# josefmaierfl/matchinglib_poselib

Hardware: AMD Instinct MI355X
Metric: descriptor-pairs/s (8k x 8k ORB BF-Hamming kNN=2 + ratio) (higher is better)
Workload: dtype fp4 (E2M1 MFMA, f32 accumulate: exact); 1 GPU; C2: 8192x8192 ORB-256 BF-Hamming kNN=2 + 0.75 ratio + DMatch rows, 64 image pair(s) per GPU per step; pairs_per_gpu=64, settle_steps=400, solver_polish=1

## Files before the change

### include/mlpl_debug.h

```cpp
#ifndef MLPL_DEBUG_H
#define MLPL_DEBUG_H
#include "mlpl_c.h"

#ifdef __cplusplus
extern "C" {
#endif

int mlpl_debug_arrsac_trace(mlpl_ctx *ctx, int32_t *buf, int cap);

int mlpl_debug_usac_trace(mlpl_ctx *ctx, double *buf, int cap_records);

int mlpl_debug_ransac_draw(mlpl_ctx *ctx, long long out[2]);

long long mlpl_debug_fiber_selftest(int n, int workers, int rounds);

int mlpl_debug_eig9(mlpl_ctx *ctx, const double *G, const double *start, int count, double *out12, double *jacobi10);

int mlpl_debug_dk_stats(mlpl_ctx *ctx, int enable, int stats[16]);

int mlpl_debug_l2_flags(mlpl_ctx *ctx, int flags[4]);

int mlpl_debug_hamming_stamps(mlpl_ctx *ctx, unsigned long long *out, int max_items);

int mlpl_debug_hamming_clock(mlpl_ctx *ctx, unsigned long long *out, int max_items);

int mlpl_debug_hop_trace(mlpl_ctx *ctx, float *us, int *codes, int max_items, long long *ws_grows);

int mlpl_debug_last_kernels(mlpl_ctx *ctx, int out[13]);

int mlpl_debug_last_hamming_top2(mlpl_ctx *ctx);

int mlpl_debug_last_l2_match(mlpl_ctx *ctx, int out[4]);

int mlpl_debug_l2_fold_counts(mlpl_ctx *ctx, const float *d_q, int nq, size_t q_stride, size_t q_batch_stride, const float *d_t, int nt,
                              size_t t_stride, size_t t_batch_stride, int dim, int ratio_test, float ratio, int batch, int32_t *d_idx, float *d_dist,
                              int32_t *counts);

int mlpl_debug_count_pass(mlpl_ctx *ctx, const double *p1, const double *p2, int n, const double *E, int n_live, int n_bound,
                          const int32_t *ids, int table_len, double thresh2, int point_splits, int32_t *table_inout);

#ifdef __cplusplus
}
#endif
#endif
```

### matchinglib_poselib_amd/_lib.py

```python
from __future__ import annotations

import ctypes as C
import os
import threading

_HERE = os.path.dirname(os.path.abspath(__file__))
_LIB_PATH = os.environ.get("MLPL_LIB_PATH") or os.path.join(_HERE, "lib", "libmlpl_hip.so")

MLPL_OK = 0
MLPL_E_BAD_INPUT = -1
MLPL_E_UNSUPPORTED = -2
MLPL_E_FAILED = -3
MLPL_E_INTERNAL = -103
MLPL_E_FEW_KEYPOINTS = -4
MLPL_E_NO_DEVICE = -100
MLPL_E_HIP = -101
MLPL_E_NOMEM = -102


class MlplError(RuntimeError):
    def __init__(self, code: int, where: str, msg: str = ""):
        self.code = code
        super().__init__(f"{where} failed with code {code}: {msg}")

# ... 77 lines not shown
    "mlpl_usac_essential_dev": (c_int, [c_void_p, c_void_p, c_void_p, c_int, c_void_p, c_void_p, c_void_p, c_void_p, c_void_p]),
    "mlpl_usac_essential_batch_dev": (c_int, [c_void_p, c_int, c_void_p, c_void_p, c_int, c_void_p, c_void_p, c_void_p, c_void_p, c_void_p, c_void_p,
                                              c_void_p, c_void_p, c_int, c_void_p, c_void_p]),
    "mlpl_usac_last_stats": (c_int, [c_void_p, c_void_p]),
    "mlpl_usac_last_degeneracy": (c_int, [c_void_p, c_void_p, c_void_p, c_void_p, c_int]),
    "mlpl_debug_usac_trace": (c_int, [c_void_p, c_void_p, c_int]),
    "mlpl_ransac_essential": (c_int, [c_void_p, c_void_p, c_void_p, c_int, c_double, c_double, c_int, c_int, c_u32,
                                      c_void_p, c_void_p, C.POINTER(c_int), C.POINTER(c_int)]),
    "mlpl_ransac_essential_dev": (c_int, [c_void_p, c_void_p, c_void_p, c_int, c_double, c_double, c_int, c_int,
                                          c_u32, c_void_p, c_void_p, C.POINTER(c_int), C.POINTER(c_int), c_void_p]),
    "mlpl_solve_5pt": (c_int, [c_void_p, c_void_p, c_void_p, c_int, c_void_p, c_int, c_void_p, c_void_p]),
    "mlpl_score_models": (c_int, [c_void_p, c_void_p, c_void_p, c_int, c_void_p, c_int, c_double, c_void_p,
                                  c_void_p]),
    "mlpl_ransac_last_stats": (c_int, [c_void_p, c_void_p]),
    "mlpl_debug_ransac_draw": (c_int, [c_void_p, c_void_p]),
    "mlpl_debug_fiber_selftest": (C.c_longlong, [c_int, c_int, c_int]),
    "mlpl_debug_eig9": (c_int, [c_void_p, c_void_p, c_void_p, c_int, c_void_p, c_void_p]),
    "mlpl_debug_dk_stats": (c_int, [c_void_p, c_int, c_void_p]),
    "mlpl_debug_hamming_stamps": (c_int, [c_void_p, c_void_p, c_int]),
    "mlpl_debug_hamming_clock": (c_int, [c_void_p, c_void_p, c_int]),
    "mlpl_debug_hop_trace": (c_int, [c_void_p, c_void_p, c_void_p, c_int, c_void_p]),
    "mlpl_debug_last_kernels": (c_int, [c_void_p, c_void_p]),
    "mlpl_debug_last_hamming_top2": (c_int, [c_void_p]),
    "mlpl_debug_count_pass": (c_int, [c_void_p, c_void_p, c_void_p, c_int, c_void_p, c_int, c_int, c_void_p, c_int, c_double, c_int,
                                      c_void_p]),
    "mlpl_pair_pose_dev": (c_int, [c_void_p, c_void_p, c_int, c_void_p, c_int, c_int, c_void_p, c_void_p, c_void_p, c_void_p, c_double,
                                   c_int, c_double, c_int, c_u32, c_double, c_void_p, c_void_p]),
    "mlpl_pair_pose_batch_dev": (c_int, [c_void_p, c_int, c_void_p, c_int, c_void_p, c_int, c_int, c_void_p, c_void_p, c_void_p, c_void_p, c_double,
                                         c_int, c_double, c_int, c_void_p, c_double, c_void_p, c_void_p, c_void_p]),
    "mlpl_pair_pose_f32_dev": (c_int, [c_void_p, c_void_p, c_int, c_void_p, c_int, c_int, c_void_p, c_void_p, c_void_p, c_void_p, c_double,
                                       c_int, c_double, c_int, c_u32, c_double, c_void_p, c_void_p]),
    "mlpl_pair_pose_batch_f32_dev": (c_int, [c_void_p, c_int, c_void_p, c_int, c_void_p, c_int, c_int, c_void_p, c_void_p, c_void_p, c_void_p, c_double,
                                             c_int, c_double, c_int, c_void_p, c_double, c_void_p, c_void_p, c_void_p]),
    "mlpl_pair_pose_batch_usac_f32_dev": (c_int, [c_void_p, c_int, c_void_p, c_int, c_void_p, c_int, c_int, c_void_p, c_void_p, c_void_p, c_void_p, c_void_p, c_int,
                                                  c_void_p, c_double, c_void_p, c_void_p, c_void_p]),
    "mlpl_pair_pose_batch_arrsac_f32_dev": (c_int, [c_void_p, c_int, c_void_p, c_int, c_void_p, c_int, c_int, c_void_p, c_void_p, c_void_p, c_void_p, c_double, c_int,
                                                    c_void_p, c_double, c_void_p, c_void_p, c_void_p]),
    "mlpl_pair_pose_batch_lanes_dev": (c_int, [c_void_p, c_void_p, c_int, c_int, c_void_p, c_int, c_void_p, c_int, c_int, c_void_p, c_void_p, c_void_p, c_void_p,
                                               c_double, c_int, c_double, c_void_p, c_double, c_void_p, c_void_p, c_void_p]),
    "mlpl_pair_pose_batch_usac_dev": (c_int, [c_void_p, c_int, c_void_p, c_int, c_void_p, c_int, c_int, c_void_p, c_void_p, c_void_p, c_void_p, c_void_p, c_int,
                                              c_void_p, c_double, c_void_p, c_void_p, c_void_p]),
    "mlpl_pair_pose_batch_arrsac_dev": (c_int, [c_void_p, c_int, c_void_p, c_int, c_void_p, c_int, c_int, c_void_p, c_void_p, c_void_p, c_void_p, c_double, c_int,
                                                c_void_p, c_double, c_void_p, c_void_p, c_void_p]),
    "mlpl_sorted_match_idx": (c_int, [c_void_p, c_int, c_void_p]),
    "mlpl_pair_batch_last_stats": (c_int, [c_void_p, c_void_p]),
    "mlpl_ransac_essential_batch_dev": (c_int, [c_void_p, c_int, c_void_p, c_void_p, c_int, c_void_p, c_double, c_int, c_double, c_void_p, c_int, c_double,
# ... 118 lines not shown
        check(self._lib.mlpl_ctx_synchronize(self._h), "mlpl_ctx_synchronize")

    def set_option(self, name: str, value: int):
        check(self._lib.mlpl_set_option(self._h, name.encode(), int(value)), "mlpl_set_option")

    def get_option(self, name: str) -> int:
        v = C.c_int(0)
        check(self._lib.mlpl_get_option(self._h, name.encode(), C.byref(v)), "mlpl_get_option")
        return v.value

    def last_kernels(self) -> list:
        out = (C.c_int * 13)()
        n = self._lib.mlpl_debug_last_kernels(self._h, out)
        if n < 0:
            raise MlplError(n, "mlpl_debug_last_kernels", last_error())
        return list(out[:n])

    def last_hamming_top2(self) -> int:
        n = self._lib.mlpl_debug_last_hamming_top2(self._h)
        if n < 0:
            raise MlplError(n, "mlpl_debug_last_hamming_top2", last_error())
        return n

    def last_l2_match(self) -> list:
        out = (C.c_int * 4)()
        n = self._lib.mlpl_debug_last_l2_match(self._h, out)
        if n < 0:
            raise MlplError(n, "mlpl_debug_last_l2_match", last_error())
        return list(out[:n])

    def close(self):
        if getattr(self, "_h", None) is not None and self._h:
            self._lib.mlpl_ctx_destroy(self._h)
            self._h = None

    def __del__(self):
        try:
            self.close()
        except Exception:
            pass

    def __enter__(self):
        return self

    def __exit__(self, *exc):
        self.close()
# ... 15 lines not shown
```

### matchinglib_poselib_amd/csrc/capi.hip

```cpp

#include <algorithm>
#include <cfloat>
#include <cstdlib>
#include <cstring>
#include <new>

#include "mlpl_internal.h"

namespace mlpl {

static thread_local char g_err[512] = "";

void set_error(const char *fmt, ...) {
    va_list ap;
    va_start(ap, fmt);
    vsnprintf(g_err, sizeof(g_err), fmt, ap);
    va_end(ap);
}

int ws_get(mlpl_ctx *ctx, WsSlot slot, size_t bytes, void **out) {
    if (bytes < 4096) bytes = 4096;
    if (ctx->ws_bytes[slot] < bytes) {
        MLPL_HIP_TRY(hipDeviceSynchronize());
        if (ctx->ws[slot]) MLPL_HIP_TRY(hipFree(ctx->ws[slot]));
// ... 91 lines not shown
    hipDeviceProp_t prop;
    MLPL_HIP_TRY(hipGetDeviceProperties(&prop, device_ordinal));
    if (std::strncmp(prop.gcnArchName, "gfx950", 6) != 0) {
        set_error("device %d is %s; this library carries gfx950 code objects only", device_ordinal, prop.gcnArchName);
        return MLPL_E_NO_DEVICE;
    }
    mlpl_ctx *ctx = new (std::nothrow) mlpl_ctx();
    if (!ctx) return MLPL_E_NOMEM;
    std::memset(ctx, 0, sizeof(*ctx));
    ctx->device = device_ordinal;
    ctx->num_cus = prop.multiProcessorCount > 0 ? prop.multiProcessorCount : 256;
    ctx->opt_hamming_variant = 3;
    ctx->opt_hamming_qpl = 1;
    ctx->opt_hamming_blocks_per_cu = 32;
    ctx->opt_hamming_mfma_blocks_per_cu = 3;
    ctx->opt_hamming_mfma_qt = 0;
    ctx->opt_hamming_mfma_lds = 1;
    ctx->opt_hamming_mfma_weighted = 1;
    ctx->opt_hamming_mfma_prio = 0;
    ctx->opt_hamming_fused_merge = 1;
    ctx->opt_hamming_expand_fine = 1;
    ctx->opt_hamming_expand_inkernel = 1;
    ctx->opt_hamming_block_top2 = 4;
    ctx->opt_hamming_merge_emit = 0;
    ctx->opt_ransac_lazy_sums = 1;
    ctx->opt_ransac_overlap = 1;
    ctx->opt_ransac_f32_filter = 1;
    ctx->opt_ransac_count_mpl = 2;
    ctx->opt_ransac_count_tiles = 2;
    ctx->opt_ransac_count_wpe = 5;
    ctx->opt_ransac_count_threads = 256;
    ctx->opt_ransac_count_defer = 1;
    ctx->opt_pair_batch_feed = 1;
    ctx->opt_solver_polish = 1;
    ctx->opt_solver_wave3 = 1;
    ctx->opt_ransac_device_draw = 1;
    ctx->opt_usac_lo_warm_start = 1;
    ctx->opt_usac_lo5_fused_fit = 1;
    ctx->opt_hub_blocking_sync = 1;
    ctx->opt_eig_inverse_iteration = 1;
    ctx->opt_arrsac_refine_warm_start = 1;
    ctx->opt_usac_sprt_fast = 1;
    ctx->opt_l2_float_mfma = 1;
    ctx->opt_l2_fold_counts = 1;
    ctx->opt_vfc_store_u = 0;
    hipError_t e = hipStreamCreateWithFlags(&ctx->stream, hipStreamNonBlocking);
// ... 41 lines not shown
    for (int i = 0; i < 2; ++i)
        if (ctx->aux_stream[i]) (void)hipStreamDestroy(ctx->aux_stream[i]);
    for (int i = 0; i < 8; ++i)
        if (ctx->aux_ev[i]) (void)hipEventDestroy(ctx->aux_ev[i]);
    delete ctx;
}

void *mlpl_ctx_stream(mlpl_ctx *ctx) { return ctx ? (void *)ctx->stream : nullptr; }
int mlpl_ctx_device(mlpl_ctx *ctx) { return ctx ? ctx->device : -1; }
int mlpl_ctx_synchronize(mlpl_ctx *ctx) {
    if (!ctx) return MLPL_E_BAD_INPUT;
    MLPL_HIP_TRY(hipStreamSynchronize(ctx->stream));
    return MLPL_OK;
}

static const struct {
    const char *name;
    int mlpl_ctx::*field;
    int lo, hi;
} kRangeOptions[] = {
    {"l2_fold_counts", &mlpl_ctx::opt_l2_fold_counts, 0, 1},
    {"hamming_expand_inkernel", &mlpl_ctx::opt_hamming_expand_inkernel, 0, 1},
    {"hamming_block_top2", &mlpl_ctx::opt_hamming_block_top2, 0, 4},
    {"vfc_store_u", &mlpl_ctx::opt_vfc_store_u, 0, 1},
};

int mlpl_set_option(mlpl_ctx *ctx, const char *name, int value) {
    if (!ctx || !name) return MLPL_E_BAD_INPUT;
    for (const auto &o : kRangeOptions)
        if (!std::strcmp(name, o.name)) {
            const bool bad_block = o.field == &mlpl_ctx::opt_hamming_block_top2 && value != 0 && value != 4;
            if (value < o.lo || value > o.hi || bad_block) {
                set_error("mlpl_set_option: unknown option or bad value: %s=%d", name, value);
                return MLPL_E_BAD_INPUT;
            }
            ctx->*(o.field) = value;
            return MLPL_OK;
        }
    if (!std::strcmp(name, "hamming_variant") && value >= 0 && value <= 3) ctx->opt_hamming_variant = value;
    else if (!std::strcmp(name, "hamming_mfma_qt") && (value == 0 || value == 1 || value == 2 || value == 4)) ctx->opt_hamming_mfma_qt = value;
    else if (!std::strcmp(name, "hamming_mfma_blocks_per_cu") && value >= 1 && value <= 64) ctx->opt_hamming_mfma_blocks_per_cu = value;
    else if (!std::strcmp(name, "hamming_mfma_lds") && (value >= 0 && value <= 2)) ctx->opt_hamming_mfma_lds = value;
    else if (!std::strcmp(name, "hamming_expand_fine") && (value == 0 || value == 1)) ctx->opt_hamming_expand_fine = value;
    else if (!std::strcmp(name, "hamming_mfma_prio") && (value == 0 || value == 1 || value == 3)) ctx->opt_hamming_mfma_prio = value;
    else if (!std::strcmp(name, "hamming_mfma_prefetch") && (value == 0 || value == 2 || value == 4 || value == 6)) ctx->opt_hamming_mfma_prefetch = value;
    else if (!std::strcmp(name, "hamming_split_rows") && (value == 0 || value == 4096 || value == 8192)) ctx->opt_hamming_split_rows = value;
    else if (!std::strcmp(name, "hamming_mfma_waves") && (value == 0 || value == 4 || value == 8 || value == 16)) ctx->opt_hamming_mfma_waves = value;
    else if (!std::strcmp(name, "hamming_mfma_weighted") && (value == 0 || value == 1)) ctx->opt_hamming_mfma_weighted = value;
    else if (!std::strcmp(name, "hamming_fused_merge") && (value == 0 || value == 1)) ctx->opt_hamming_fused_merge = value;
    else if (!std::strcmp(name, "hamming_stamps") && (value >= 0 && value <= 2)) ctx->opt_hamming_stamps = value;
    else if (!std::strcmp(name, "hamming_train01") && (value == 0 || value == 1)) ctx->opt_hamming_train01 = value;
    else if (!std::strcmp(name, "hamming_merge_emit") && (value == 0 || value == 1)) ctx->opt_hamming_merge_emit = value;
    else if (!std::strcmp(name, "l2_mfma_waves") && (value == 0 || value == 4 || value == 8)) ctx->opt_l2_mfma_waves = value;
    else if (!std::strcmp(name, "l2_mfma_blocks_per_cu") && value >= 0 && value <= 16) ctx->opt_l2_mfma_blocks_per_cu = value;
    else if (!std::strcmp(name, "hamming_qpl") && (value == 1 || value == 2)) ctx->opt_hamming_qpl = value;
// ... 91 lines not shown
    else if (!std::strcmp(name, "pair_batch_raw_cap")) *value = ctx->opt_pair_batch_raw_cap;
    else if (!std::strcmp(name, "usac_lo_stepwise")) *value = ctx->opt_usac_lo_stepwise;
    else if (!std::strcmp(name, "usac_lo_warm_start")) *value = ctx->opt_usac_lo_warm_start;
    else if (!std::strcmp(name, "usac_first_batch")) *value = ctx->opt_usac_first_batch;
    else if (!std::strcmp(name, "usac_lo5_fused_fit")) *value = ctx->opt_usac_lo5_fused_fit;
    else if (!std::strcmp(name, "usac_sprt_fast")) *value = ctx->opt_usac_sprt_fast;
    else if (!std::strcmp(name, "ransac_host_table")) *value = ctx->opt_ransac_host_table;
    else if (!std::strcmp(name, "ransac_chunk")) *value = ctx->opt_ransac_chunk;
    else {
        set_error("mlpl_get_option: unknown option: %s", name);
        return MLPL_E_BAD_INPUT;
    }
    return MLPL_OK;
}

int mlpl_debug_last_kernels(mlpl_ctx *ctx, int out[13]) {
    if (!ctx || !out) return MLPL_E_BAD_INPUT;
    out[0] = ctx->dbg_count_kernel[0], out[1] = ctx->dbg_count_kernel[1];
    for (int i = 0; i < 11; ++i) out[2 + i] = ctx->dbg_hamming_kernel[i];
    return 13;
}

int mlpl_debug_last_hamming_top2(mlpl_ctx *ctx) { return ctx ? ctx->dbg_hamming_top2 : MLPL_E_BAD_INPUT; }

int mlpl_debug_last_l2_match(mlpl_ctx *ctx, int out[4]) {
    if (!ctx || !out) return MLPL_E_BAD_INPUT;
    for (int i = 0; i < 4; ++i) out[i] = ctx->dbg_l2_match[i];
    return 4;
}

int mlpl_debug_hamming_stamps(mlpl_ctx *ctx, unsigned long long *out, int max_items) {
    if (!ctx || !out) return MLPL_E_BAD_INPUT;
    MLPL_HIP_TRY(hipSetDevice(ctx->device));
    MLPL_HIP_TRY(hipDeviceSynchronize());
    if (max_items < 0) {
        const int n = ctx->dbg_stamp_items < -max_items ? ctx->dbg_stamp_items : -max_items;
        if (n > 0 && ctx->ws[WS_DEBUG])
            MLPL_HIP_TRY(hipMemcpy(out, (char *)ctx->ws[WS_DEBUG] + (size_t)ctx->dbg_stamp_items * 32, (size_t)n * 48 * 8, hipMemcpyDeviceToHost));
        return n;
    }
    const int n = ctx->dbg_stamp_items < max_items ? ctx->dbg_stamp_items : max_items;
    if (n > 0 && ctx->ws[WS_DEBUG]) MLPL_HIP_TRY(hipMemcpy(out, ctx->ws[WS_DEBUG], (size_t)n * 32, hipMemcpyDeviceToHost));
    return n;
}

int mlpl_debug_hop_trace(mlpl_ctx *ctx, float *us, int *codes, int max_items, long long *ws_grows) {
// ... 608 lines not shown
```

### matchinglib_poselib_amd/csrc/knn_hamming.hip

```cpp

#include "mlpl_internal.h"

namespace mlpl {

namespace {

constexpr int kQueriesPerBlock = 256;
constexpr int kTileRows = 128;
constexpr int kMergeGroup = 64;
static_assert(kMergeGroup == kCountGroup, "merge kernel and ratio_write_kernel disagree on the count granularity");

constexpr int dist_bits(int nw) {
    int b = 1;
    while ((1 << b) <= nw * 32) ++b;
    return b;
}

__device__ __forceinline__ uint32_t bcnt_acc(uint32_t x, uint32_t acc) {
    uint32_t r;
    asm("v_bcnt_u32_b32 %0, %1, %2" : "=v"(r) : "v"(x), "v"(acc));
    return r;
}

__device__ __forceinline__ uint32_t umed3(uint32_t a, uint32_t b, uint32_t c) {
// ... 433 lines not shown
    const int max_split = (nt + kTileRows - 1) / kTileRows;
    long long want = (target_blocks + (long long)qtiles * batch - 1) / ((long long)qtiles * batch);
    int nsplit = (int)std::max<long long>(1, std::min<long long>(want, max_split));
    int rps = (nt + nsplit - 1) / nsplit;
    rps = ((rps + kTileRows - 1) / kTileRows) * kTileRows;
    const int max_rps = ((1 << dshift) - 2) / kTileRows * kTileRows;
    if (rps > max_rps) rps = max_rps;
    nsplit = (nt + rps - 1) / rps;
    if (nsplit > 65535) {
        set_error("knn_hamming: train set too large (nt=%d)", nt);
        return MLPL_E_BAD_INPUT;
    }

    void *part = nullptr;
    int rc = ws_get(ctx, WS_PARTIAL, (size_t)batch * nsplit * nq * sizeof(uint2), &part);
    if (rc) return rc;

    dim3 grid(qtiles, nsplit, batch);
    {
        int *rec = ctx->dbg_hamming_kernel;
        rec[0] = variant, rec[1] = (variant == 1 && nw <= 16) ? qpl : 1, rec[2] = 0, rec[3] = 0, rec[4] = 0;
        rec[5] = 0, rec[6] = 0, rec[7] = 0, rec[8] = nsplit, rec[9] = 0, rec[10] = 0;
        ctx->dbg_hamming_top2 = 0;
    }
    prof_mark(ctx, MLPL_PROF_KNN_HAMMING, 0, s);
    switch (nw) {
        case 1: launch_partial<1>(variant, qpl, grid, s, qw, qbw, tw, tbw, nq, nt, rps, nsplit, (uint2 *)part); break;
        case 2: launch_partial<2>(variant, qpl, grid, s, qw, qbw, tw, tbw, nq, nt, rps, nsplit, (uint2 *)part); break;
        case 4: launch_partial<4>(variant, qpl, grid, s, qw, qbw, tw, tbw, nq, nt, rps, nsplit, (uint2 *)part); break;
        case 8: launch_partial<8>(variant, qpl, grid, s, qw, qbw, tw, tbw, nq, nt, rps, nsplit, (uint2 *)part); break;
        case 16: launch_partial<16>(variant, qpl, grid, s, qw, qbw, tw, tbw, nq, nt, rps, nsplit, (uint2 *)part); break;
        case 32: launch_partial<32>(variant, qpl, grid, s, qw, qbw, tw, tbw, nq, nt, rps, nsplit, (uint2 *)part); break;
        case 64: launch_partial<64>(variant, qpl, grid, s, qw, qbw, tw, tbw, nq, nt, rps, nsplit, (uint2 *)part); break;
        default: set_error("knn_hamming: unsupported descriptor width %d bytes", nbytes); return MLPL_E_BAD_INPUT;
    }
    prof_mark(ctx, MLPL_PROF_KNN_HAMMING, 1, s);
    launch_merge(s, (const uint2 *)part, nq, nsplit, rps, dshift, k, ratio, batch, d_idx, d_dist, d_group_counts);
    MLPL_HIP_TRY(hipGetLastError());
    return MLPL_OK;
}

}
```

### matchinglib_poselib_amd/csrc/knn_hamming_mfma.hip

```cpp

#include <algorithm>
#include <cmath>
#include <type_traits>
#include <vector>

#include "mlpl_internal.h"


namespace mlpl {

namespace {

typedef int v8i __attribute__((ext_vector_type(8)));
typedef float v16f __attribute__((ext_vector_type(16)));
typedef uint32_t u32x4 __attribute__((ext_vector_type(4)));
typedef uint32_t u32x2 __attribute__((ext_vector_type(2)));

constexpr float kEps = 1.0f / 16384.0f;
constexpr int kMaxRowsPerSplit = 8192;
constexpr float kAccBias = 704.0f;
static_assert(kAccBias == (float)(int)kAccBias, "the bias is an integer: rint() of a value is kAccBias + I");
static_assert(kAccBias + 256.0f + (float)(kMaxRowsPerSplit - 32) / 16384.0f < 1024.0f, "largest value (identical rows, last tile) below 2^10: 2^-14 is exact");
static_assert(kAccBias - 256.0f - 31.0f / 16384.0f > -1024.0f, "smallest value (complementary rows) above -2^10");
static_assert(kAccBias - 64.0f >= 512.0f && kAccBias + 64.0f < 1024.0f, "typical data (|I| <= 64) stay inside the binade [512, 1024)");
// ... 709 lines not shown
                        const int d1 = (int32_t)(b1 >> 32);
                        fuse.idx[o + 1] = (int32_t)(b1 & 0xFFFFFFFFull);
                        fuse.dist[o + 1] = d1;
                        pass = (float)d0 < __fmul_rn(fuse.ratio, (float)d1);
                    } else {
                        pass = true;
                    }
                }
                const int c = __popcll(__ballot(pass));
                const int q_wave = q_first + rr * (64 * NW) + (int)(tid_end & ~63u);
                if (fuse.group_counts && le == 0 && q_wave < nq && rr * (64 * NW) + (int)(tid_end & ~63u) < NW * QT * 32) fuse.group_counts[(size_t)b * ((nq + 63) >> 6) + (q_wave >> 6)] = c;
            }
        }
    }
    if (stamps && l_end == 0) clock_stamp(stamps + ((size_t)item * NW + w) * 4, st_c, st_r, ntiles, QT);
    if (fuse.clk && item == 0 && tid_end == 0) {
        fuse.clk[0] = __builtin_amdgcn_s_memtime() - st_c;
        fuse.clk[1] = __builtin_amdgcn_s_memrealtime() - st_r;
        fuse.clk[2] = st_r;
        fuse.clk[3] = fuse.launch_no;
    }
}

template <int QT>
__global__ __launch_bounds__(256, 4) void knn_hamming_mfma_dyn_kernel(
    const uint4 *__restrict__ qfrag, size_t q_batch_u4, const uint4 *__restrict__ tfrag, size_t t_batch_u4, int nq, int nt,
    int span_tiles, int nspan, int nmem, int chunk_tiles, int dshift, int qblocks, int n_items, uint2 *__restrict__ part,
    int *__restrict__ counters, unsigned long long *__restrict__ stamps) {
    constexpr int KS = 4, NB = 3;
    __shared__ __attribute__((aligned(16))) uint4 ring[NB][KS * 64];
    __shared__ int s_claim, s_first;
    const int l = threadIdx.x & 63;
    const int w = __builtin_amdgcn_readfirstlane((int)(threadIdx.x >> 6));
    unsigned long long st_c = 0, st_r = 0;
    clock_start(stamps != nullptr, st_c, st_r);
    const int item = xcd_block_item();
    if (item >= n_items) return;
    const int slots = nspan * nmem;
    const int qb = item % qblocks;
    const int slot_id = (item / qblocks) % slots;
    const int b = item / (qblocks * slots);
    const int span = slot_id / nmem;
    int *ctr = counters + ((size_t)b * qblocks + qb) * nspan + span;
    const int qt0 = (qb * 4 + w) * QT;
    const uint4 *qf = qfrag + (size_t)b * q_batch_u4 + (size_t)qt0 * KS * 64 + l;

// ... 128 lines not shown
        default: f(int_c<8>{}); break;
    }
}

struct RingLaunch {
    dim3 grid;
    hipStream_t s;
    const uint32_t *qw;
    size_t q_batch_words;
    const void *tsrc;
    size_t t_batch;
    int nq, nt, rps, nsplit, dshift, qblocks, n_items;
    uint2 *part;
    unsigned long long *stamps;
    const int32_t *split_tab;
    HammingFuse fuse;
};
template <int QT, int PRIO, int NW = 4, int PD = 2, bool XP = false, bool ST = false, int BT = 0>
void launch_ring(const RingLaunch &a) {
    hipLaunchKernelGGL((knn_hamming_mfma_lds_kernel<QT, PRIO, NW, PD, XP, ST, BT>), a.grid, dim3(64 * NW), 0, a.s, a.qw, a.q_batch_words, a.tsrc,
                       a.t_batch, a.nq, a.nt, a.rps, a.nsplit, a.dshift, a.qblocks, a.n_items, a.part, a.stamps, a.split_tab, a.fuse);
}

bool age_aware_split_table(unsigned grid_x, long long items, int num_cus, int qblocks, int nsplit, int batch, int t_tiles, int max_rps,
                           std::vector<int32_t> &tab) {
    const int per_xcd = (int)(grid_x >> 3);
    tab.assign((size_t)batch * (nsplit + 1), -1);
    for (long long bid = 0; bid < items; ++bid) {
        const long long item = (bid & 7) * per_xcd + (bid >> 3);
        if (item >= items) continue;
        const int sp = (int)((item / qblocks) % nsplit), bb = (int)(item / ((long long)qblocks * nsplit));
        const int r = (int)(bid / num_cus);
        int32_t &slot = tab[(size_t)bb * (nsplit + 1) + sp];
        if (slot < 0) slot = r;
        else if (slot != r) return false;
    }
    static const double kRate[4] = {1.0 / 1700, 1.0 / 2100, 1.0 / 3200, 1.0 / 5300};
    for (int bb = 0; bb < batch; ++bb) {
        int32_t *h = tab.data() + (size_t)bb * (nsplit + 1);
        double wsum = 0;
        for (int sp = 0; sp < nsplit; ++sp) wsum += kRate[h[sp]];
        int acc_tiles = 0;
        double acc_w = 0;
        for (int sp = 0; sp < nsplit; ++sp) {
            acc_w += kRate[h[sp]];
            h[sp] = acc_tiles;
// ... 59 lines not shown
        nmem = (int)std::max<long long>(1, std::min<long long>(want_mem, (span_tiles + chunk_tiles - 1) / chunk_tiles));
        nsplit = nspan * nmem;
        rps = span_tiles * 32;
        sps = nmem;
        if (nsplit > 65535) {
            set_error("knn_hamming: train set too large (nt=%d)", nt);
            return MLPL_E_BAD_INPUT;
        }
    }
    const long long items = (lds_ring ? (long long)qblocks : (long long)qgroups) * nsplit * batch;
    if (items > (1LL << 30)) {
        set_error("knn_hamming: problem too large for one launch (nq=%d nt=%d batch=%d)", nq, nt, batch);
        return MLPL_E_BAD_INPUT;
    }

    const int pd = (nwv == 8 && (ctx->opt_hamming_mfma_prefetch == 4 || ctx->opt_hamming_mfma_prefetch == 6)) ? ctx->opt_hamming_mfma_prefetch : 2;
    const int prio = (nwv == 16 || pd != 2) ? 0 : ctx->opt_hamming_mfma_prio == 1 ? 1 : (ctx->opt_hamming_mfma_prio == 3 && nwv == 8) ? 3 : 0;
    const int train01 = (lds_ring && !dyn && ctx->opt_hamming_train01) ? 1 : 0;
    const bool inkernel = ctx->opt_hamming_expand_inkernel && lds_ring && !dyn && nwv == 8 && pd == 2 && prio == 0 && nw == 8 && !train01 &&
                          ((uintptr_t)tw & 3u) == 0;

    const int block_top2 = inkernel ? ctx->opt_hamming_block_top2 : 0;
    ctx->dbg_hamming_top2 = block_top2;

    void *qf = nullptr, *tf = nullptr, *part = nullptr;
    int rc;
    const size_t q_u4 = (size_t)q_tiles_padded * ks * 64, t_u4 = (size_t)t_tiles * ks * 64;
    if ((rc = ws_get(ctx, WS_FRAG_Q, (size_t)batch * q_u4 * 16, &qf))) return rc;
    if (!inkernel && (rc = ws_get(ctx, WS_FRAG_T, ((size_t)batch * t_u4 + (size_t)ks * 64) * 16, &tf))) return rc;
    if ((rc = ws_get(ctx, WS_PARTIAL, (size_t)batch * nsplit * nq * sizeof(uint2), &part))) return rc;
    int *counters = nullptr;
    const int counters_per_batch = dyn ? qblocks * nspan : 0;
    if (dyn) {
        void *cp = nullptr;
        if ((rc = ws_get(ctx, WS_COUNTERS, (size_t)batch * counters_per_batch * sizeof(int), &cp))) return rc;
        counters = (int *)cp;
    }
    const bool expand_q = !(lds_ring && !dyn);
    const ExpandArgs ta{tw, t_batch_words, nt, t_tiles, (uint4 *)tf};
    const ExpandArgs qa = expand_q ? ExpandArgs{qw, q_batch_words, nq, q_tiles_padded, (uint4 *)qf} : ta;
    const dim3 egrid((unsigned)(((expand_q ? std::max(q_tiles_padded, t_tiles) : t_tiles) * 64 + 255) / 256), batch, expand_q ? 2 : 1);
    const bool expand_fine = !inkernel && !expand_q && ks == 4 && nw == 8 && !counters && (long long)t_tiles * batch <= 4LL * ctx->num_cus && ctx->opt_hamming_expand_fine;
    if (inkernel) {
    } else if (expand_fine) {
        hipLaunchKernelGGL(hamming_expand_fine_kernel, dim3((unsigned)t_tiles, batch), dim3(256), 0, s, ta, train01);
    } else {
// ... 51 lines not shown
        *fused_out = 1;
    }
    {
        int *rec = ctx->dbg_hamming_kernel;
        rec[0] = dyn ? 5 : lds_ring ? 4 : 3, rec[1] = (dyn || !lds_ring) ? (ks <= 4 && qt == 4 ? 4 : qt >= 2 ? 2 : 1) : qt;
        rec[2] = (lds_ring && !dyn) ? prio : 0, rec[3] = lds_ring && !dyn ? nwv : 4, rec[4] = lds_ring && !dyn ? pd : 0;
        rec[5] = *fused_out, rec[6] = split_tab != nullptr, rec[7] = expand_fine, rec[8] = nsplit, rec[9] = ks, rec[10] = inkernel;
    }
    prof_mark(ctx, MLPL_PROF_KNN_HAMMING, 0, s);
    if (dyn) {
        auto launch_dyn = [&](auto QT) {
            hipLaunchKernelGGL((knn_hamming_mfma_dyn_kernel<decltype(QT)::value>), grid, dim3(256), 0, s, (const uint4 *)qf, q_u4, (const uint4 *)tf, t_u4, nq,
                               nt, span_tiles, nspan, nmem, chunk_tiles, dshift, qblocks, (int)items, (uint2 *)part, counters, stamps);
        };
        if (qt == 4) launch_dyn(int_c<4>{});
        else if (qt == 2) launch_dyn(int_c<2>{});
        else launch_dyn(int_c<1>{});
    } else if (lds_ring) {
        const RingLaunch ra{grid, s, qw, q_batch_words, inkernel ? (const void *)tw : (const void *)tf, inkernel ? t_batch_words : t_u4, nq, nt, rps, nsplit,
                            dshift, qblocks, (int)items, (uint2 *)part, stamps, split_tab, fuse};
        if (inkernel && stamps)
            block_top2 == 4 ? launch_ring<4, 0, 8, 2, true, true, 4>(ra) : launch_ring<4, 0, 8, 2, true, true>(ra);
        else if (inkernel)
            block_top2 == 4 ? launch_ring<4, 0, 8, 2, true, false, 4>(ra) : launch_ring<4, 0, 8, 2, true>(ra);
        else if (nwv == 16) launch_ring<4, 0, 16>(ra);
        else if (nwv == 8 && pd == 4) launch_ring<4, 0, 8, 4>(ra);
        else if (nwv == 8 && pd == 6) launch_ring<4, 0, 8, 6>(ra);
        else if (nwv == 8 && prio == 3) launch_ring<4, 3, 8>(ra);
        else if (nwv == 8 && prio == 1) launch_ring<4, 1, 8>(ra);
        else if (nwv == 8) launch_ring<4, 0, 8>(ra);
        else if (qt == 4) prio == 1 ? launch_ring<4, 1>(ra) : launch_ring<4, 0>(ra);
        else if (qt == 2) prio == 1 ? launch_ring<2, 1>(ra) : launch_ring<2, 0>(ra);
        else prio == 1 ? launch_ring<1, 1>(ra) : launch_ring<1, 0>(ra);
    } else {
        dispatch_ks(ks, [&](auto KS) {
            auto launch_mfma = [&](auto QT) {
                hipLaunchKernelGGL((knn_hamming_mfma_kernel<decltype(KS)::value, decltype(QT)::value>), grid, dim3(256), 0, s, (const uint4 *)qf, q_u4,
                                   (const uint4 *)tf, t_u4, nq, nt, rps, nsplit, dshift, qgroups, (int)items, (uint2 *)part, stamps);
            };
            if constexpr (decltype(KS)::value <= 4) {
                if (qt == 4) return launch_mfma(int_c<4>{});
            }
            if (qt >= 2) launch_mfma(int_c<2>{});
            else launch_mfma(int_c<1>{});
        });
    }
    prof_mark(ctx, MLPL_PROF_KNN_HAMMING, 1, s);
// ... 11 lines not shown
```

### matchinglib_poselib_amd/csrc/mlpl_internal.h

```cpp
#pragma once

#include <hip/hip_runtime.h>

#include <cstdarg>
#include <cstddef>
#include <cstdint>
#include <cstdio>

#include "mlpl_c.h"
#include "mlpl_debug.h"

namespace mlpl {

void set_error(const char *fmt, ...);

#define MLPL_HIP_TRY(expr)                                                                                  \
    do {                                                                                                    \
        hipError_t e__ = (expr);                                                                            \
        if (e__ != hipSuccess) {                                                                            \
            ::mlpl::set_error("%s:%d: %s -> %s", __FILE__, __LINE__, #expr, hipGetErrorString(e__));        \
            return MLPL_E_HIP;                                                                              \
        }                                                                                                   \
    } while (0)

// ... 86 lines not shown
    int opt_hamming_mfma_qt;
    int opt_hamming_mfma_lds;
    int opt_hamming_mfma_waves;
    int opt_hamming_split_rows;
    int opt_hamming_mfma_prefetch;
    int opt_hamming_mfma_prio;
    int opt_hamming_mfma_weighted;
    long long split_tab_key;
    void *split_tab_ptr;
    int opt_hamming_fused_merge;
    void *hamming_tickets_ptr;
    size_t hamming_tickets_bytes;
    int opt_hamming_expand_fine;
    int opt_hamming_stamps;
    long long hamming_clock_launches;
    int opt_hamming_merge_emit;
    void *hamming_scan_ptr;
    size_t hamming_scan_bytes;
    uint32_t hamming_scan_gen;
    int opt_hamming_train01;
    int opt_vfc_store_u;
    int opt_hamming_expand_inkernel;
    int opt_hamming_block_top2;
    int dbg_hamming_top2;
    void *subpix_sep_mask_ptr;
    int dbg_stamp_items;
    int dbg_count_kernel[2];
    int dbg_hamming_kernel[11];
    int opt_ransac_chunk;
    int opt_ransac_event_cap;
    int opt_ransac_count_mpl;
    int opt_ransac_count_threads;
    int opt_ransac_count_wpe;
    int opt_ransac_count_tiles;
    int opt_ransac_count_defer;
    int opt_ransac_f32_filter;
    int opt_ransac_overlap;
    int opt_ransac_dev_split;
    int opt_ransac_lazy_sums;
    int opt_solver_polish;
    int opt_solver_wave3;
    int opt_ransac_host_table;
    int opt_rand_cache_max;
    void *rand_cache;
    int32_t *ransac_T_host;
    int ransac_T_n;
// ... 184 lines not shown
```

Before: 13190 billion descriptor-pairs/s.

## Add 16x16x128 FP4 MFMA ring kernel for Hamming top-2 path

Adds a new Hamming kNN kernel that uses 16x16x128 f8f6f4 MFMA instructions instead of the 32-row shape. It keeps the LDS ring with in-kernel bit-plane expansion, tracks top-2 per 16-row half with med3/max3, and rescans within a 4-row block for the second best. Split results are folded through a ticket scheme. A new option selects this kernel and defaults to 16, so it replaces the existing block_top2=4 in-kernel path. The aim is higher MFMA throughput or lower register pressure, at the cost of a large hand-scheduled asm kernel that carries correctness risk.

Result: faster. 13420 billion descriptor-pairs/s (median of 6 runs) (+1.7%).

```diff
diff --git a/include/mlpl_debug.h b/include/mlpl_debug.h
--- a/include/mlpl_debug.h
+++ b/include/mlpl_debug.h
@@ -30,6 +30,8 @@
 
 int mlpl_debug_last_hamming_top2(mlpl_ctx *ctx);
 
+int mlpl_debug_last_hamming_shape(mlpl_ctx *ctx);
+
 int mlpl_debug_last_l2_match(mlpl_ctx *ctx, int out[4]);
 
 int mlpl_debug_l2_fold_counts(mlpl_ctx *ctx, const float *d_q, int nq, size_t q_stride, size_t q_batch_stride, const float *d_t, int nt,
diff --git a/matchinglib_poselib_amd/_lib.py b/matchinglib_poselib_amd/_lib.py
--- a/matchinglib_poselib_amd/_lib.py
+++ b/matchinglib_poselib_amd/_lib.py
@@ -123,6 +123,7 @@
     "mlpl_debug_hop_trace": (c_int, [c_void_p, c_void_p, c_void_p, c_int, c_void_p]),
     "mlpl_debug_last_kernels": (c_int, [c_void_p, c_void_p]),
     "mlpl_debug_last_hamming_top2": (c_int, [c_void_p]),
+    "mlpl_debug_last_hamming_shape": (c_int, [c_void_p]),
     "mlpl_debug_count_pass": (c_int, [c_void_p, c_void_p, c_void_p, c_int, c_void_p, c_int, c_int, c_void_p, c_int, c_double, c_int,
                                       c_void_p]),
     "mlpl_pair_pose_dev": (c_int, [c_void_p, c_void_p, c_int, c_void_p, c_int, c_int, c_void_p, c_void_p, c_void_p, c_void_p, c_double,
@@ -287,6 +288,12 @@
             raise MlplError(n, "mlpl_debug_last_hamming_top2", last_error())
         return n
 
+    def last_hamming_shape(self) -> int:
+        n = self._lib.mlpl_debug_last_hamming_shape(self._h)
+        if n < 0:
+            raise MlplError(n, "mlpl_debug_last_hamming_shape", last_error())
+        return n
+
     def last_l2_match(self) -> list:
         out = (C.c_int * 4)()
         n = self._lib.mlpl_debug_last_l2_match(self._h, out)
diff --git a/matchinglib_poselib_amd/csrc/capi.hip b/matchinglib_poselib_amd/csrc/capi.hip
--- a/matchinglib_poselib_amd/csrc/capi.hip
+++ b/matchinglib_poselib_amd/csrc/capi.hip
@@ -137,6 +137,7 @@
     ctx->opt_hamming_expand_fine = 1;
     ctx->opt_hamming_expand_inkernel = 1;
     ctx->opt_hamming_block_top2 = 4;
+    ctx->opt_hamming_mfma_shape = 16;
     ctx->opt_hamming_merge_emit = 0;
     ctx->opt_ransac_lazy_sums = 1;
     ctx->opt_ransac_overlap = 1;
@@ -224,6 +225,7 @@
     {"l2_fold_counts", &mlpl_ctx::opt_l2_fold_counts, 0, 1},
     {"hamming_expand_inkernel", &mlpl_ctx::opt_hamming_expand_inkernel, 0, 1},
     {"hamming_block_top2", &mlpl_ctx::opt_hamming_block_top2, 0, 4},
+    {"hamming_mfma_shape", &mlpl_ctx::opt_hamming_mfma_shape, 16, 32},
     {"vfc_store_u", &mlpl_ctx::opt_vfc_store_u, 0, 1},
 };
 
@@ -232,7 +234,8 @@
     for (const auto &o : kRangeOptions)
         if (!std::strcmp(name, o.name)) {
             const bool bad_block = o.field == &mlpl_ctx::opt_hamming_block_top2 && value != 0 && value != 4;
-            if (value < o.lo || value > o.hi || bad_block) {
+            const bool bad_shape = o.field == &mlpl_ctx::opt_hamming_mfma_shape && value != 16 && value != 32;
+            if (value < o.lo || value > o.hi || bad_block || bad_shape) {
                 set_error("mlpl_set_option: unknown option or bad value: %s=%d", name, value);
                 return MLPL_E_BAD_INPUT;
             }
@@ -370,6 +373,7 @@
 }
 
 int mlpl_debug_last_hamming_top2(mlpl_ctx *ctx) { return ctx ? ctx->dbg_hamming_top2 : MLPL_E_BAD_INPUT; }
+int mlpl_debug_last_hamming_shape(mlpl_ctx *ctx) { return ctx ? ctx->dbg_hamming_shape : MLPL_E_BAD_INPUT; }
 
 int mlpl_debug_last_l2_match(mlpl_ctx *ctx, int out[4]) {
     if (!ctx || !out) return MLPL_E_BAD_INPUT;
diff --git a/matchinglib_poselib_amd/csrc/knn_hamming.hip b/matchinglib_poselib_amd/csrc/knn_hamming.hip
--- a/matchinglib_poselib_amd/csrc/knn_hamming.hip
+++ b/matchinglib_poselib_amd/csrc/knn_hamming.hip
@@ -479,6 +479,7 @@
         rec[0] = variant, rec[1] = (variant == 1 && nw <= 16) ? qpl : 1, rec[2] = 0, rec[3] = 0, rec[4] = 0;
         rec[5] = 0, rec[6] = 0, rec[7] = 0, rec[8] = nsplit, rec[9] = 0, rec[10] = 0;
         ctx->dbg_hamming_top2 = 0;
+        ctx->dbg_hamming_shape = 0;
     }
     prof_mark(ctx, MLPL_PROF_KNN_HAMMING, 0, s);
     switch (nw) {
diff --git a/matchinglib_poselib_amd/csrc/knn_hamming_mfma.hip b/matchinglib_poselib_amd/csrc/knn_hamming_mfma.hip
--- a/matchinglib_poselib_amd/csrc/knn_hamming_mfma.hip
+++ b/matchinglib_poselib_amd/csrc/knn_hamming_mfma.hip
@@ -755,6 +755,368 @@
     }
 }
 
+typedef float v4f __attribute__((ext_vector_type(4)));
+static_assert(kAccBias + 256.0f + 32.0f / 16384.0f < 1024.0f, "a chain of a pair's first tile starts 32 eps higher: still below 2^10");
+
+template <int QPB, int THREADS>
+__device__ __forceinline__ void fold_splits_by_ticket(const HammingFuse &fuse, uint2 *__restrict__ part, const int32_t *__restrict__ split_tile0, int b, int qb,
+                                                      int qblocks, int nsplit, int rows_per_split, int nq, int dshift, unsigned tid_end, int le) {
+    __shared__ int s_last;
+    asm volatile("s_waitcnt vmcnt(0)" ::: "memory");
+    __syncthreads();
+    if (tid_end == 0) {
+        const int old = __hip_atomic_fetch_add(&fuse.tickets[(size_t)b * qblocks + qb], 1, __ATOMIC_RELAXED, __HIP_MEMORY_SCOPE_AGENT);
+        s_last = old == nsplit - 1;
+        if (s_last) __hip_atomic_store(&fuse.tickets[(size_t)b * qblocks + qb], 0, __ATOMIC_RELAXED, __HIP_MEMORY_SCOPE_AGENT);
+    }
+    __syncthreads();
+    if (s_last) {
+        const uint32_t lmask = (1u << dshift) - 1u;
+        const int q_first = qb * QPB;
+#pragma unroll 1
+        for (int rr = 0; rr * THREADS < QPB; ++rr) {
+            const int ql = rr * THREADS + (int)tid_end;
+            const int q = ql < QPB ? q_first + ql : nq;
+            unsigned long long b0 = ~0ull, b1 = ~0ull;
+            auto upd = [&](unsigned long long g) {
+                const bool lt0 = g < b0, lt1 = g < b1;
+                b1 = lt0 ? b0 : (lt1 ? g : b1);
+                b0 = lt0 ? g : b0;
+            };
+            bool pass = false;
+            if (q < nq) {
+                for (int sp = 0; sp < nsplit; ++sp) {
+                    const unsigned long long pw = __hip_atomic_load(reinterpret_cast<const unsigned long long *>(&part[((size_t)b * nsplit + sp) * nq + q]),
+                                                                    __ATOMIC_RELAXED, __HIP_MEMORY_SCOPE_AGENT);
+                    const uint2 pv = make_uint2((uint32_t)pw, (uint32_t)(pw >> 32));
+                    const unsigned long long base = split_tile0 ? 32ull * (unsigned long long)split_tile0[(size_t)b * (nsplit + 1) + sp]
+                                                                : (unsigned long long)sp * rows_per_split;
+                    if (pv.x != 0xFFFFFFFFu) upd(((unsigned long long)(pv.x >> dshift) << 32) | (base + (pv.x & lmask)));
+                    if (pv.y != 0xFFFFFFFFu) upd(((unsigned long long)(pv.y >> dshift) << 32) | (base + (pv.y & lmask)));
+                }
+                const size_t o = ((size_t)b * nq + q) * fuse.k;
+                const int d0 = (int32_t)(b0 >> 32);
+                fuse.idx[o] = (int32_t)(b0 & 0xFFFFFFFFull);
+                fuse.dist[o] = d0;
+                if (fuse.k == 2) {
+                    const int d1 = (int32_t)(b1 >> 32);
+                    fuse.idx[o + 1] = (int32_t)(b1 & 0xFFFFFFFFull);
+                    fuse.dist[o + 1] = d1;
+                    pass = (float)d0 < __fmul_rn(fuse.ratio, (float)d1);
+                } else {
+                    pass = true;
+                }
+            }
+            const int c = __popcll(__ballot(pass));
+            const int q_wave = q_first + rr * THREADS + (int)(tid_end & ~63u);
+            if (fuse.group_counts && le == 0 && q_wave < nq && rr * THREADS + (int)(tid_end & ~63u) < QPB) fuse.group_counts[(size_t)b * ((nq + 63) >> 6) + (q_wave >> 6)] = c;
+        }
+    }
+}
+
+__device__ __forceinline__ void mfma16_group(const u32x4 (&a)[4], const u32x4 &q0, const u32x4 &q1, const v4f &ci0, const v4f &ci1, v4f &c0, v4f &c1) {
+    asm volatile("v_mfma_f32_16x16x128_f8f6f4 %0, %2, %6, %8 cbsz:4 blgp:4\n\t"
+                 "v_mfma_f32_16x16x128_f8f6f4 %1, %4, %6, %9 cbsz:4 blgp:4\n\t"
+                 "v_mfma_f32_16x16x128_f8f6f4 %0, %3, %7, %0 cbsz:4 blgp:4\n\t"
+                 "v_mfma_f32_16x16x128_f8f6f4 %1, %5, %7, %1 cbsz:4 blgp:4\n\t"
+                 "s_nop 7"
+                 : "=&v"(c0), "=&v"(c1)
+                 : "v"(a[0]), "v"(a[1]), "v"(a[2]), "v"(a[3]), "v"(q0), "v"(q1), "v"(ci0), "v"(ci1));
+}
+template <bool REBASE>
+__device__ __forceinline__ void top2_update_halves(float &m1, float &m2, const v4f &c0, const v4f &c1, float step) {
+    const float g0 = __builtin_fmaxf(__builtin_fmaxf(__builtin_fmaxf(c0[0], c0[1]), c0[2]), c0[3]);
+    const float g1 = __builtin_fmaxf(__builtin_fmaxf(__builtin_fmaxf(c1[0], c1[1]), c1[2]), c1[3]);
+    float sec;
+    if constexpr (REBASE)
+        asm volatile("v_add_f32 %0, %5, %0\n\tv_add_f32 %1, %5, %1\n\tv_med3_f32 %2, %0, %3, %4\n\tv_max3_f32 %0, %0, %3, %4\n\tv_max_f32 %1, %1, %2"
+                     : "+v"(m1), "+v"(m2), "=&v"(sec) : "v"(g0), "v"(g1), "s"(step));
+    else
+        asm volatile("v_med3_f32 %2, %0, %3, %4\n\tv_max3_f32 %0, %0, %3, %4\n\tv_max_f32 %1, %1, %2" : "+v"(m1), "+v"(m2), "=&v"(sec) : "v"(g0), "v"(g1));
+}
+__device__ __forceinline__ uint2 top2_across_groups(const uint32_t (&k)[2]) {
+    uint32_t k0 = k[0], k1 = k[1];
+#pragma unroll
+    for (int x = 16; x <= 32; x <<= 1) {
+        const uint32_t o0 = __shfl_xor(k0, x), o1 = __shfl_xor(k1, x);
+        k1 = umed3(k0, k1, o0);
+        k0 = min(k0, o0);
+        k1 = umed3(k0, k1, o1);
+        k0 = min(k0, o1);
+    }
+    return make_uint2(k0, k1);
+}
+__device__ __forceinline__ uint32_t block_rescan4(uint32_t k0, const uint32_t (&q8)[8], const char *rbase, int rows, int dshift, int g) {
+    const uint32_t lmask = (1u << dshift) - 1u;
+    const int best = (int)(k0 & lmask);
+    const int r = (best & ~3) + g;
+    const RawRow t = *reinterpret_cast<const RawRow *>(rbase + (size_t)min(r, rows - 1) * 32);
+    int d = 0;
+#pragma unroll
+    for (int j = 0; j < 8; ++j) d += __popc(t.w[j] ^ q8[j]);
+    const uint32_t key = ((uint32_t)d << dshift) | (uint32_t)r;
+    uint32_t res = (r != best && r < rows && k0 != 0xFFFFFFFFu) ? key : 0xFFFFFFFFu;
+    res = min(res, (uint32_t)__shfl_xor(res, 16));
+    return min(res, (uint32_t)__shfl_xor(res, 32));
+}
+
+__global__ __launch_bounds__(64 * 8, 4) void knn_hamming_mfma_lds16_kernel(
+    const uint32_t *__restrict__ qw, size_t q_batch_words, const void *__restrict__ tsrc, size_t t_batch, int nq, int nt,
+    int rows_per_split, int nsplit, int dshift, int qblocks, int n_items, uint2 *__restrict__ part,
+    unsigned long long *__restrict__ stamps, const int32_t *__restrict__ split_tile0, HammingFuse fuse) {
+    constexpr int QT = 4, NG = 2 * QT, NW = 8, PD = 2, KS = 4, NR = 4;
+    __shared__ __attribute__((aligned(16))) uint4 ring[2][KS * 64];
+    __shared__ __attribute__((aligned(16))) uint32_t raw_ring[NR * 256];
+    const int l = threadIdx.x & 63;
+    const int w = __builtin_amdgcn_readfirstlane((int)(threadIdx.x >> 6));
+    unsigned long long st_c = 0, st_r = 0;
+    clock_start(stamps || fuse.clk, st_c, st_r);
+    const int item = xcd_block_item();
+    if (item >= n_items) return;
+    const int qb = item % qblocks;
+    const int split = (item / qblocks) % nsplit;
+    const int b = item / (qblocks * nsplit);
+    const int qt0 = (qb * NW + w) * QT;
+
+    u32x4 bq[NG][2];
+    v4f cinit[2][2];
+#pragma unroll
+    for (int J = 0; J < 2; ++J)
+#pragma unroll
+        for (int rh = 0; rh < 2; ++rh)
+#pragma unroll
+            for (int i = 0; i < 4; ++i) cinit[J][rh][i] = kAccBias + (float)((J == 0 ? 32 : 0) - (16 * rh + 4 * (l >> 4) + i)) * kEps;
+
+    int row0 = split * rows_per_split;
+    int row1 = min(nt, row0 + rows_per_split);
+    if (split_tile0) {
+        row0 = 32 * split_tile0[(size_t)b * (nsplit + 1) + split];
+        row1 = min(nt, 32 * split_tile0[(size_t)b * (nsplit + 1) + split + 1]);
+    }
+    const int tile0 = row0 >> 5;
+    const int ntiles = (row1 - row0 + 31) >> 5;
+
+    float m1[NG], m2[NG];
+#pragma unroll
+    for (int u = 0; u < NG; ++u) m1[u] = m2[u] = -INFINITY;
+
+    const char *rbase = (const char *)tsrc + ((size_t)b * t_batch + (size_t)tile0 * 32 * (2 * KS)) * 4;
+    const uint32_t raw_last = (uint32_t)(nt - row0) * (8u * KS) - 4u;
+    uint32_t xp_frag, xp_raw, xp_plane, xp_voff;
+    int xp_it0 = 0;
+    auto copy_tile = [&](int t_rel) {
+        if (w >= KS) return;
+        const uint32_t off = min(xp_voff + (uint32_t)(t_rel - PD - xp_it0) * 1024u, raw_last);
+        __builtin_amdgcn_global_load_lds((const void *)(rbase + off),
+                                         (__attribute__((address_space(3))) void *)&raw_ring[((t_rel + NR - 1) & (NR - 1)) * 256 + w * 64], 4, 0, 0);
+    };
+    const uint32_t raw_lds = (uint32_t)(uintptr_t)(__attribute__((address_space(3))) uint32_t *)&raw_ring[0];
+    const uint32_t frag_lds = (uint32_t)(uintptr_t)(__attribute__((address_space(3))) uint4 *)&ring[0][0];
+    {
+        const uint32_t lx = (uint32_t)l;
+        xp_frag = frag_lds + lx * 16u;
+        xp_raw = raw_lds + (uint32_t)w * 4u + (lx >> 1) * 32u;
+        xp_plane = frag_lds + (lx >> 5) * 2048u + (uint32_t)(w >> 2) * 1024u + (uint32_t)(w & 3) * 256u + (lx & 31u) * 8u;
+        xp_voff = PD * 1024u + (uint32_t)w * 256u + lx * 4u;
+        asm volatile("" : "+v"(xp_frag), "+v"(xp_raw), "+v"(xp_plane), "+v"(xp_voff));
+    }
+    auto raw_addr = [&](int t_rel) { return xp_raw + (uint32_t)((t_rel + NR - 1) & (NR - 1)) * 1024u; };
+    auto plane_addr = [&](int t_rel) { return xp_plane + (uint32_t)(t_rel & 1) * (KS * 1024u); };
+    auto expand_pair = [&](uint32_t x) {
+        const uint32_t y = x >> __builtin_amdgcn_ubfe(xp_plane, 3u, 1u);
+        return u32x2{expand_plane0(y, 0x22222222u), expand_plane2(y, 0x22222222u)};
+    };
+    auto tile_math = [&](const u32x4 (&r)[KS], const v4f (&c)[2], auto rebase) {
+        constexpr int RB = decltype(rebase)::value;
+#pragma unroll
+        for (int u = 0; u < NG; ++u) {
+            v4f c0, c1;
+            mfma16_group(r, bq[u][0], bq[u][1], c[0], c[1], c0, c1);
+            top2_update_halves<RB != 0>(m1[u], m2[u], c0, c1, (float)RB * kEps);
+            __builtin_amdgcn_sched_barrier(0);
+        }
+    };
+    auto tile_body = [&](int it, const v4f (&c)[2]) {
+        u32x4 r[KS];
+        uint32_t x;
+        const uint32_t addr = xp_frag + (uint32_t)(it & 1) * (KS * 1024u);
+        const uint32_t ra = raw_addr(it + 1), wa = plane_addr(it + 1);
+        asm volatile(
+            "ds_read_b32 %4, %6\n\tds_read_b128 %0, %5\n\tds_read_b128 %1, %5 offset:1024\n\tds_read_b128 %2, %5 offset:2048\n\t"
+            "ds_read_b128 %3, %5 offset:3072"
+            : "=&v"(r[0]), "=&v"(r[1]), "=&v"(r[2]), "=&v"(r[3]), "=&v"(x)
+            : "v"(addr), "v"(ra)
+            : "memory");
+        asm volatile("s_waitcnt lgkmcnt(4)" : "+v"(x));
+        const u32x2 o = expand_pair(x);
+        asm volatile("ds_write_b64 %0, %1" ::"v"(wa), "v"(o) : "memory");
+        asm volatile("s_waitcnt lgkmcnt(4)" : "+v"(r[0]));
+        asm volatile("s_waitcnt lgkmcnt(3)" : "+v"(r[1]));
+        asm volatile("s_waitcnt lgkmcnt(2)" : "+v"(r[2]));
+        asm volatile("s_waitcnt lgkmcnt(1)" : "+v"(r[3]));
+        tile_math(r, c, std::integral_constant<int, 32>{});
+    };
+
+#pragma unroll
+    for (int t = 0; t < PD; ++t)
+        if (t < ntiles) copy_tile(t);
+#pragma unroll
+    for (int u = 0; u < NG; ++u) {
+        const int row = qt0 * 32 + 16 * u + (l & 15);
+        uint32_t v0 = 0u, v1 = 0u;
+        if (row < nq) {
+            const uint32_t *qp = qw + (size_t)b * q_batch_words + (size_t)row * (2 * KS) + (size_t)(l >> 4);
+            v0 = qp[0], v1 = qp[KS];
+        }
+        bq[u][0] = u32x4{expand_plane(v0, 0), expand_plane(v0, 2), expand_plane(v0, 1), expand_plane(v0, 3)};
+        bq[u][1] = u32x4{expand_plane(v1, 0), expand_plane(v1, 2), expand_plane(v1, 1), expand_plane(v1, 3)};
+    }
+    {
+        asm volatile("s_waitcnt vmcnt(0)" ::: "memory");
+        __builtin_amdgcn_s_barrier();
+        uint32_t x;
+        asm volatile("ds_read_b32 %0, %1\n\ts_waitcnt lgkmcnt(0)" : "=&v"(x) : "v"(raw_addr(0)) : "memory");
+        const u32x2 o = expand_pair(x);
+        asm volatile("ds_write_b64 %0, %1" ::"v"(plane_addr(0)), "v"(o) : "memory");
+    }
+
+    const bool ragged = row0 + ntiles * 32 > nt;
+    const int nfull = ragged ? ntiles - 1 : ntiles;
+    auto arrive = [&](int it) {
+        if (it + PD < ntiles) {
+            copy_tile(it + PD);
+            asm volatile("s_waitcnt vmcnt(1) lgkmcnt(0)" ::: "memory");
+        } else {
+            asm volatile("s_waitcnt vmcnt(0) lgkmcnt(0)" ::: "memory");
+        }
+        __builtin_amdgcn_s_barrier();
+    };
+    int it = 0;
+    {
+        const uint32_t dma_lds = raw_lds + (uint32_t)w * 256u;
+        int raw_step = 2 * 1024;
+        auto tile_fixed = [&](auto jc, auto copier) {
+            constexpr int J = decltype(jc)::value;
+            __builtin_amdgcn_sched_barrier(0);
+            if constexpr (decltype(copier)::value) {
+                const uint32_t m0 = dma_lds + (uint32_t)((it + J + PD + NR - 1) & (NR - 1)) * 1024u - (uint32_t)J * 1024u;
+                __builtin_amdgcn_global_load_lds((const void *)(rbase + xp_voff), (__attribute__((address_space(3))) void *)(uintptr_t)m0, 4, J * 1024, 0);
+            }
+            asm volatile("s_waitcnt vmcnt(1) lgkmcnt(0)" ::: "memory");
+            __builtin_amdgcn_s_barrier();
+            u32x4 r[KS];
+            uint32_t x;
+            asm volatile(
+                "ds_read_b32 %4, %6 offset:%7\n\tds_read_b128 %0, %5 offset:%8\n\tds_read_b128 %1, %5 offset:%8+1024\n\t"
+                "ds_read_b128 %2, %5 offset:%8+2048\n\tds_read_b128 %3, %5 offset:%8+3072"
+                : "=&v"(r[0]), "=&v"(r[1]), "=&v"(r[2]), "=&v"(r[3]), "=&v"(x)
+                : "v"(xp_frag), "v"(xp_raw), "i"(J * 1024), "i"((J & 1) * (KS * 1024))
+                : "memory");
+            asm volatile("s_waitcnt lgkmcnt(4)" : "+v"(x));
+            const u32x2 o = expand_pair(x);
+            asm volatile("ds_write_b64 %0, %1 offset:%2" ::"v"(xp_plane), "v"(o), "i"(((J + 1) & 1) * (KS * 1024)) : "memory");
+            asm volatile("s_waitcnt lgkmcnt(4)" : "+v"(r[0]));
+            asm volatile("s_waitcnt lgkmcnt(3)" : "+v"(r[1]));
+            asm volatile("s_waitcnt lgkmcnt(2)" : "+v"(r[2]));
+            asm volatile("s_waitcnt lgkmcnt(1)" : "+v"(r[3]));
+            tile_math(r, cinit[J], std::integral_constant<int, J == 0 ? 64 : 0>{});
+        };
+        auto run_pairs = [&](auto copier) {
+            while (it + 3 < nfull) {
+                tile_fixed(std::integral_constant<int, 0>{}, copier);
+                tile_fixed(std::integral_constant<int, 1>{}, copier);
+                if constexpr (decltype(copier)::value) xp_voff += 2 * 1024, xp_it0 += 2;
+                xp_raw += (uint32_t)raw_step;
+                raw_step = -raw_step;
+                it += 2;
+            }
+        };
+        if (w < KS) run_pairs(std::true_type{});
+        else run_pairs(std::false_type{});
+        if (raw_step < 0) xp_raw -= 2 * 1024;
+    }
+    for (; it < nfull; ++it) {
+        arrive(it);
+        tile_body(it, cinit[1]);
+    }
+    const int l_end = (int)__builtin_amdgcn_mbcnt_hi(~0u, __builtin_amdgcn_mbcnt_lo(~0u, 0u));
+    const unsigned tid_end = (unsigned)(w * 64 + l_end);
+    if (ragged) {
+        arrive(nfull);
+#pragma unroll
+        for (int rh = 0; rh < 2; ++rh)
+#pragma unroll
+            for (int i = 0; i < 4; ++i) {
+                const int lr = 16 * rh + 4 * (l_end >> 4) + i;
+                cinit[1][rh][i] = (row0 + nfull * 32 + lr < nt) ? kAccBias - (float)lr * kEps : -INFINITY;
+            }
+        tile_body(nfull, cinit[1]);
+    }
+
+    int le = l_end, qt0e = qt0;
+    asm volatile("" : "+v"(le), "+s"(qt0e));
+    const int ge = le >> 4;
+    const float frame = (float)(32 * (ntiles - 1));
+    int pass_acc = 0;
+#pragma unroll
+    for (int u = 0; u < NG; ++u) {
+        uint32_t k[2];
+        const float mm[2] = {m1[u], m2[u]};
+#pragma unroll
+        for (int j = 0; j < 2; ++j)
+            k[j] = mm[j] == -INFINITY ? 0xFFFFFFFFu : decode_key_biased(mm[j], frame, dshift, DistRule{64 * KS, 0, 0});
+        const uint2 kk = top2_across_groups(k);
+        const int q = qt0e * 32 + 16 * u + (le & 15);
+        const uint32_t k0 = kk.x;
+        uint32_t k1 = kk.y;
+        if (fuse.k != 1) {
+            uint32_t q8[8] = {0u, 0u, 0u, 0u, 0u, 0u, 0u, 0u};
+            if (q < nq) {
+                const uint4 *qp = reinterpret_cast<const uint4 *>(qw + (size_t)b * q_batch_words + (size_t)q * (2 * KS));
+                const uint4 v0 = qp[0], v1 = qp[1];
+                q8[0] = v0.x, q8[1] = v0.y, q8[2] = v0.z, q8[3] = v0.w, q8[4] = v1.x, q8[5] = v1.y, q8[6] = v1.z, q8[7] = v1.w;
+            }
+            k1 = min(k1, block_rescan4(k0, q8, rbase, nt - row0, dshift, ge));
+        }
+        if (fuse.idx && nsplit == 1) {
+            const uint32_t lmask = (1u << dshift) - 1u;
+            bool pass = false;
+            if (ge == 0 && q < nq) {
+                const size_t o = ((size_t)b * nq + q) * fuse.k;
+                const int d0 = k0 == 0xFFFFFFFFu ? -1 : (int)(k0 >> dshift);
+                fuse.idx[o] = k0 == 0xFFFFFFFFu ? -1 : (int)(row0 + (k0 & lmask));
+                fuse.dist[o] = d0;
+                if (fuse.k == 2) {
+                    const int d1 = k1 == 0xFFFFFFFFu ? -1 : (int)(k1 >> dshift);
+                    fuse.idx[o + 1] = k1 == 0xFFFFFFFFu ? -1 : (int)(row0 + (k1 & lmask));
+                    fuse.dist[o + 1] = d1;
+                    pass = (float)d0 < __fmul_rn(fuse.ratio, (float)d1);
+                } else {
+                    pass = true;
+                }
+            }
+            const int c = __popcll(__ballot(pass));
+            pass_acc = (u & 3) ? pass_acc + c : c;
+            if (fuse.group_counts && (u & 3) == 3 && le == 0 && qt0e * 32 + 16 * (u - 3) < nq)
+                fuse.group_counts[(size_t)b * ((nq + 63) >> 6) + ((qt0e * 32 + 16 * u) >> 6)] = pass_acc;
+        } else if (ge == 0 && q < nq) {
+            if (fuse.idx)
+                __hip_atomic_store(reinterpret_cast<unsigned long long *>(&part[((size_t)b * nsplit + split) * nq + q]),
+                                   (unsigned long long)k0 | ((unsigned long long)k1 << 32), __ATOMIC_RELAXED, __HIP_MEMORY_SCOPE_AGENT);
+            else
+                part[((size_t)b * nsplit + split) * nq + q] = make_uint2(k0, k1);
+        }
+    }
+    if (fuse.idx && nsplit > 1) fold_splits_by_ticket<NW * QT * 32, 64 * NW>(fuse, part, split_tile0, b, qb, qblocks, nsplit, rows_per_split, nq, dshift, tid_end, le);
+    if (stamps && l_end == 0) clock_stamp(stamps + ((size_t)item * NW + w) * 4, st_c, st_r, ntiles, QT);
+    if (fuse.clk && item == 0 && tid_end == 0) {
+        fuse.clk[0] = __builtin_amdgcn_s_memtime() - st_c;
+        fuse.clk[1] = __builtin_amdgcn_s_memrealtime() - st_r;
+        fuse.clk[2] = st_r;
+        fuse.clk[3] = fuse.launch_no;
+    }
+}
+
 template <int QT>
 __global__ __launch_bounds__(256, 4) void knn_hamming_mfma_dyn_kernel(
     const uint4 *__restrict__ qfrag, size_t q_batch_u4, const uint4 *__restrict__ tfrag, size_t t_batch_u4, int nq, int nt,
@@ -929,6 +1291,11 @@
                        a.t_batch, a.nq, a.nt, a.rps, a.nsplit, a.dshift, a.qblocks, a.n_items, a.part, a.stamps, a.split_tab, a.fuse);
 }
 
+void launch_ring16(const RingLaunch &a) {
+    hipLaunchKernelGGL(knn_hamming_mfma_lds16_kernel, a.grid, dim3(64 * 8), 0, a.s, a.qw, a.q_batch_words, a.tsrc, a.t_batch, a.nq, a.nt, a.rps, a.nsplit, a.dshift,
+                       a.qblocks, a.n_items, a.part, a.stamps, a.split_tab, a.fuse);
+}
+
 bool age_aware_split_table(unsigned grid_x, long long items, int num_cus, int qblocks, int nsplit, int batch, int t_tiles, int max_rps,
                            std::vector<int32_t> &tab) {
     const int per_xcd = (int)(grid_x >> 3);
@@ -1034,6 +1401,8 @@
 
     const int block_top2 = inkernel ? ctx->opt_hamming_block_top2 : 0;
     ctx->dbg_hamming_top2 = block_top2;
+    const int shape = (inkernel && block_top2 == 4 && ctx->opt_hamming_stamps != 1 && ctx->opt_hamming_mfma_shape == 16) ? 16 : 32;
+    ctx->dbg_hamming_shape = shape;
 
     void *qf = nullptr, *tf = nullptr, *part = nullptr;
     int rc;
@@ -1131,7 +1500,7 @@
         if (inkernel && stamps)
             block_top2 == 4 ? launch_ring<4, 0, 8, 2, true, true, 4>(ra) : launch_ring<4, 0, 8, 2, true, true>(ra);
         else if (inkernel)
-            block_top2 == 4 ? launch_ring<4, 0, 8, 2, true, false, 4>(ra) : launch_ring<4, 0, 8, 2, true>(ra);
+            block_top2 != 4 ? launch_ring<4, 0, 8, 2, true>(ra) : shape == 16 ? launch_ring16(ra) : launch_ring<4, 0, 8, 2, true, false, 4>(ra);
         else if (nwv == 16) launch_ring<4, 0, 16>(ra);
         else if (nwv == 8 && pd == 4) launch_ring<4, 0, 8, 4>(ra);
         else if (nwv == 8 && pd == 6) launch_ring<4, 0, 8, 6>(ra);
diff --git a/matchinglib_poselib_amd/csrc/mlpl_internal.h b/matchinglib_poselib_amd/csrc/mlpl_internal.h
--- a/matchinglib_poselib_amd/csrc/mlpl_internal.h
+++ b/matchinglib_poselib_amd/csrc/mlpl_internal.h
@@ -132,6 +132,8 @@
     int opt_vfc_store_u;
     int opt_hamming_expand_inkernel;
     int opt_hamming_block_top2;
+    int opt_hamming_mfma_shape;
+    int dbg_hamming_shape;
     int dbg_hamming_top2;
     void *subpix_sep_mask_ptr;
     int dbg_stamp_items;
```
